# ygtxr1997/CelebBasis

Hardware: NVIDIA H100
Metric: celeb-basis training steps/sec (SD-v1 UNet 512^2, bs=1/GPU) (higher is better)
Workload: dtype f16 operands / f32 accumulate+residual (reference: f32 with TF32 convs)

## Files before the change

### celebbasis_b200/_abi.py

```python
import ctypes as C

_p, _i, _l, _f = C.c_void_p, C.c_int32, C.c_longlong, C.c_float

SIGS = {
    "cb_groupnorm_cluster_plan": [_i, _i, _i, _i, _i, _p],
    "cb_groupnorm_fwd": [_p, _i, _p, _i, _p, _p, _i, _i, _i, _i, _f, _i, _p, _p, _p, _p],
    "cb_groupnorm_bwd": [_p, _i, _p, _i, _p, _p, _p, _p, _p, _i, _p, _i, _i, _i, _i, _i, _i, _p, _p],
    "cb_layernorm_fwd": [_p, _i, _p, _i, _p, _p, _i, _i, _f, _p, _p, _p],
    "cb_layernorm_bwd": [_p, _i, _p, _i, _p, _p, _p, _p, _i, _p, _i, _i, _i, _p],
    "cb_axpby2d": [_p, _i, _l, _f, _p, _i, _l, _f, _p, _i, _l, _l, _i, _p],
    "cb_act_fwd": [_p, _i, _p, _i, _l, _i, _p],
    "cb_act_bwd": [_p, _i, _p, _i, _p, _i, _l, _i, _p],
    "cb_geglu_fwd": [_p, _p, _i, _l, _i, _i, _p],
    "cb_geglu_bwd": [_p, _p, _p, _i, _i, _l, _i, _i, _p],
    "cb_softmax_fwd": [_p, _p, _i, _l, _i, _i, _i, _p],
    "cb_softmax_bwd": [_p, _p, _p, _i, _i, _l, _i, _i, _p],
    "cb_upsample2x_fwd": [_p, _p, _i, _i, _i, _i, _i, _p],
    "cb_upsample2x_bwd": [_p, _i, _p, _i, _i, _i, _i, _i, _i, _p],
    "cb_zero_insert2x": [_p, _p, _i, _i, _i, _i, _i, _p],
    "cb_nchw_to_nhwc": [_p, _p, _i, _i, _i, _i, _i, _p],
    "cb_nhwc_to_nchw": [_p, _i, _p, _i, _i, _i, _i, _p],
    "cb_mse_fwd_bwd": [_p, _p, _p, _p, _i, _i, _f, _p],
    "cb_timestep_embedding": [_p, _p, _i, _i, _i, _f, _p],
    "cb_embedding_gather": [_p, _p, _p, _i, _i, _i, _p],
    "cb_celeb_mlp_fwd": [_p, _p, _p, _p, _p, _p, _i, _i, _i, _i, _f, _p],
    "cb_celeb_basis_fwd": [_p, _p, _p, _i, _i, _i, _i, _p],
    "cb_celeb_basis_bwd": [_p, _p, _p, _i, _i, _i, _i, _p],
    "cb_celeb_mlp_bwd": [_p, _p, _p, _p, _p, _p, _p, _p, _i, _i, _i, _i, _f, _f, _p],
    "cb_embed_inject_fwd": [_p, _p, _p, _p, _p, _i, _i, _i, _p],
    "cb_embed_inject_bwd": [_p, _p, _p, _i, _i, _i, _i, _p],
    "cb_adamw_step": [_p, _p, _p, _p, _l, _f, _f, _f, _f, _f, _i, _p, _p],
    "cb_posterior_sample": [_p, _p, _p, _i, _i, _i, _f, _p],
    "cb_ddim_step": [_p, _p, _p, _p, _p, _p, _l, _f, _f, _f, _f, _f, _p],
    "cb_attention_fwd": [_p, _l, _p, _l, _p, _l, _p, _l, _p, _p, _l, _i, _i, _i, _i, _i, _i, _f, _i, _p],
    "cb_attention_bwd": [_p, _l, _p, _l, _p, _l, _p, _l, _p, _l, _p, _p, _p, _l, _p, _l, _p, _l, _i, _i, _i, _i, _i, _i, _f,
                         _i, _p],
    "cb_attention_bwd_dq": [_p, _l, _p, _l, _p, _l, _p, _l, _p, _l, _p, _p, _p, _l, _p, _l, _i, _i, _i, _i, _i, _i, _f, _i, _p],
    "cb_q_sample": [_p, _p, _p, _p, _p, _p, _i, _i, _p],
    "cb_channel_affine_act": [_p, _i, _p, _i, _p, _p, _p, _l, _i, _p],
    "cb_face_warp_resize": [_p, _p, _i, _i, _i, _i, _i, _i, _i, _p, _p],
    "cb_l2norm_rows": [_p, _p, _i, _i, _p],
    "cb_ema_rows": [_p, _p, _i, _p, _i, _i, _i, _f, _p],
    "cb_face_augment": [_p, _p, _p, _p, _p, _i, _i, _i, _i, _i, _p],
    "cb_paste_resized": [_p, _i, _i, _p, _p, _i, _i, _i, _p],
    "cb_pack_conv_weight": [_p, _p, _i, _i, _i, _i, _i, _i, _i, _p, _p],
    "cb_convert_f32": [_p, _p, _i, _l, _f, _p],
}


def declare(lib):
    for name, argtypes in SIGS.items():
        fn = getattr(lib, name)
        fn.argtypes = argtypes
        fn.restype = C.c_int
```

### celebbasis_b200/csrc/cb_gemm.cu

```cuda
#include <algorithm>
#include <stdarg.h>
#include <stdio.h>
#include <stdlib.h>
#include <string.h>

#include "cb_common.cuh"

namespace cb {

constexpr int BM = 128;
constexpr int BK = 64;
constexpr int kThreads = 384;

struct GemmParams {
    int M, N, K;
    int kchunks, taps, kw;
    int ksteps_last;
    int conv;
    int out_h, out_w, img_n;
    int box_w, box_h, box_i;
    int tiles_w, tiles_h;
    int stride, pad_top, pad_left;
    int b_tap_rows, flip_taps;
    void* D;
// ... 386 lines not shown
                for (int j = 0; j < 8; ++j) {
                    fv[j] += p.bias ? s_bias[vcol + j] : 0.f;
                    fg[j] += p.bias ? s_bias[vcol + 32 + j] : 0.f;
                }
                if (p.D) {
                    store8_any(p.D, p.d_dtype, grow * p.ldd + n0 + vcol, fv);
                    store8_any(p.D, p.d_dtype, grow * p.ldd + n0 + vcol + 32, fg);
                }
                float h[8];
#pragma unroll
                for (int j = 0; j < 8; ++j) h[j] = fv[j] * gelu_f(fg[j]);
                store8_any(p.D2, p.d2_dtype, grow * p.ldd2 + ((n0 + (q >> 2) * 64) >> 1) + (q & 3) * 8, h);
            }
            return;
        }
    }

    const bool r_pre = p.R && p.vec_ok && !p.d_transposed;
    uint4 rq[kResAhead + 1][2];
    auto res_fetch = [&](int k, uint4 (&v)[2]) {
        const int u = tid + k * kThreads;
        if (u >= BM * G) return;
        const int row = u / G, col = (u % G) * 8;
        const long long grow = s_grow[row];
        if (grow >= 0 && col + 8 <= ncols_tile) residual_load8(p, r_off + grow * p.ldr + n0 + col, v);
    };
    if (r_pre) {
#pragma unroll
        for (int k = 0; k < kResAhead; ++k) res_fetch(k, rq[k]);
    }
    const int nunits = (BM * G - tid + kThreads - 1) / kThreads;
#pragma unroll 1
    for (int k = 0; k < nunits; ++k) {
        if (r_pre) res_fetch(k + kResAhead, rq[kResAhead]);
        const int u = tid + k * kThreads;
        const int row = p.d_transposed ? u % BM : u / G;
        const int col = (p.d_transposed ? u / BM : u % G) * 8;
        const long long grow = s_grow[row];
        if (col < ncols_tile && grow >= 0) {
            const int ncols = min(8, ncols_tile - col);
            float f[8], r[8];
            stage_ld8(stage + row * kPitch + col, p.alpha, f);
            if (r_pre && ncols == 8) residual_unpack8(p, rq[0], r);
            epilogue_group8<kExt>(p, f, grow, s_brow[row], n0 + col, d_off, r_off, ncols, r_pre && ncols == 8 ? r : nullptr,
                                  sbias_of(row, col));
        }
        if (dbg && k == 0 && tid == 64) dbg[6] = clock64();
        if (r_pre) {
#pragma unroll
            for (int j = 0; j < kResAhead; ++j) { rq[j][0] = rq[j + 1][0]; rq[j][1] = rq[j + 1][1]; }
        }
    }
}

template <int BN, bool A_MN, bool B_MN, int kStages, bool kExt>
__global__ void __launch_bounds__(kThreads, 1)
cb_gemm_kernel(const __grid_constant__ CUtensorMap tmA, const __grid_constant__ CUtensorMap tmB,
               const __grid_constant__ GemmParams p) {
    using Cfg = TileCfg<BN, kStages>;
    using SCfg = StageCfg<BN>;
    extern __shared__ uint8_t smem_raw[];
    const uint32_t smem_base = (smem_u32(smem_raw) + 1023u) & ~1023u;
    float* stage = reinterpret_cast<float*>(smem_raw + (smem_base - smem_u32(smem_raw)));
    const uint32_t bar_base = smem_base + kStages * Cfg::kStageBytes;
    auto full_bar = [&](int s) { return bar_base + 8u * s; };
    auto empty_bar = [&](int s) { return bar_base + 8u * (kStages + s); };

    __shared__ long long s_grow[BM];
    __shared__ int s_brow[BM];
    __shared__ __align__(16) float s_bias[BN];
    const int warp = threadIdx.x >> 5;
    const int wg = __shfl_sync(0xffffffffu, warp >> 2, 0);
    if (p.dbg_mode == 3) { pdl_sync(); return; }
    unsigned long long* dbg = p.dbg ? p.dbg + 8ull * ((blockIdx.z * gridDim.y + blockIdx.y) * gridDim.x + blockIdx.x) : nullptr;
    if (dbg && threadIdx.x == 0) { dbg[0] = clock64(); dbg[7] = gtimer(); }
    const int n0 = blockIdx.x * BN;
    const int m_tile = blockIdx.y;
    const int sp = blockIdx.z % p.splits;
    const int bz = blockIdx.z / p.splits;
    const int zi = bz % p.batch_inner;
    const int zo = bz / p.batch_inner;

    int m0 = 0, ow0 = 0, oh0 = 0, img0 = 0;
    if (p.conv) {
        const int tw = m_tile % p.tiles_w;
        const int th = (m_tile / p.tiles_w) % p.tiles_h;
        const int ti = m_tile / (p.tiles_w * p.tiles_h);
        ow0 = tw * p.box_w;
        oh0 = th * p.box_h;
        img0 = ti * p.box_i;
    } else {
        m0 = m_tile * BM;
    }

    if (threadIdx.x == 0) {
        tma_prefetch_desc(&tmA);
        tma_prefetch_desc(&tmB);
        for (int s = 0; s < kStages; ++s) {
            mbar_init(full_bar(s), 1);
            mbar_init(empty_bar(s), 8);
        }
        mbar_fence_init();
        fence_proxy_async_smem();
    }
    __syncthreads();
    if (dbg && threadIdx.x == 0) dbg[1] = clock64();
    pdl_sync();

    const int kiters_all = p.dbg_mode == 1 ? 0 : p.taps * p.kchunks;
    const int it0 = sp * p.kiters_per_split;
    const int it1 = min(kiters_all, it0 + p.kiters_per_split);

    if (wg == 0) {
        if (threadIdx.x == 0) {
            int s = 0;
            uint32_t ph = 0;
            int tap = it0 / p.kchunks;
            int kc = it0 - tap * p.kchunks;
            int r = tap / p.kw;
            int sx = tap - r * p.kw;
            for (int it = it0; it < it1; ++it) {
                mbar_wait(empty_bar(s), ph ^ 1u);
                mbar_arrive_expect_tx(full_bar(s), p.a_bytes + p.b_bytes);
                const uint32_t a_dst = smem_base + s * Cfg::kStageBytes;
                const uint32_t b_dst = a_dst + Cfg::kABytes;
                const int tap_b = p.flip_taps ? (p.taps - 1 - tap) : tap;
                if (p.conv) {
                    tma_load_4d(a_dst, &tmA, full_bar(s), kc * BK, ow0 * p.stride + sx - p.pad_left,
                                oh0 * p.stride + r - p.pad_top, img0);
                } else if (A_MN) {
                    tma_load_4d(a_dst, &tmA, full_bar(s), m0, kc * BK, zi, zo);
                    tma_load_4d(a_dst + 8192, &tmA, full_bar(s), m0 + 64, kc * BK, zi, zo);
                } else {
                    tma_load_4d(a_dst, &tmA, full_bar(s), kc * BK, m0, zi, zo);
                }
                if (B_MN) {
#pragma unroll
                    for (int j = 0; j < BN / 64; ++j)
                        tma_load_4d(b_dst + j * 8192, &tmB, full_bar(s), n0 + j * 64,
                                    tap_b * p.b_tap_rows + kc * BK, zi, zo);
                } else {
                    tma_load_4d(b_dst, &tmB, full_bar(s), kc * BK, tap_b * p.b_tap_rows + n0, zi, zo);
                }
                if (++s == kStages) { s = 0; ph ^= 1u; }
                if (++kc == p.kchunks) {
                    kc = 0;
                    ++tap;
                    if (++sx == p.kw) { sx = 0; ++r; }
                }
            }
        }
        __syncwarp();
        const int r = threadIdx.x;
        long long grow;
        bool row_valid;
        if (p.conv) {
            const int per_img = p.box_h * p.box_w;
            const int bi = r / per_img;
            const int rem = r - bi * per_img;
            const int bh = rem / p.box_w;
            const int bw = rem - bh * p.box_w;
            const int img = img0 + bi, oh = oh0 + bh, ow = ow0 + bw;
            row_valid = (bi < p.box_i) && (img < p.img_n) && (oh < p.out_h) && (ow < p.out_w);
            grow = ((long long)img * p.out_h + oh) * p.out_w + ow;
        } else {
            grow = m0 + r;
            row_valid = grow < p.M;
        }
        s_grow[r] = row_valid ? grow : -1;
        if (p.bias) {
            const long long tile_row0 = p.conv ? (((long long)img0 * p.out_h + oh0) * p.out_w + ow0) : (long long)m0;
            const long long brow0 = p.bias_row_div > 0 ? tile_row0 / p.bias_row_div : 0;
            const long long brow = p.bias_row_div > 0 ? grow / p.bias_row_div : 0;
            s_brow[r] = brow == brow0 ? -1 : static_cast<int>(brow);
            const int ncols = min(BN, p.N - n0);
            for (int i = r; i < BN; i += 128) s_bias[i] = i < ncols ? p.bias[brow0 * p.ldbias + n0 + i] : 0.f;
        }
    } else {
        float acc[BN / 2];
#pragma unroll
        for (int i = 0; i < BN / 2; ++i) acc[i] = 0.f;
        const uint32_t a_half = static_cast<uint32_t>(wg - 1) * 8192u;
        const bool releaser = (threadIdx.x & 31) == 0;
        int s = 0, s_prev = 0;
        uint32_t ph = 0;
        int kc = it0 % p.kchunks;
        for (int it = it0; it < it1; ++it) {
            mbar_wait(full_bar(s), ph);
            if (dbg && it == it0 && threadIdx.x == 128) dbg[2] = clock64();
            const uint32_t a_src = smem_base + s * Cfg::kStageBytes + a_half;
            const uint32_t b_src = smem_base + s * Cfg::kStageBytes + Cfg::kABytes;
            const int ksteps = (kc == p.kchunks - 1) ? p.ksteps_last : (BK / 16);
            wgmma_fence_regs(acc);
            if (p.bf16) mma_kiter<BN, A_MN, B_MN, true>(acc, a_src, b_src, ksteps);
            else mma_kiter<BN, A_MN, B_MN, false>(acc, a_src, b_src, ksteps);
            wgmma_wait<1>();
            wgmma_fence_regs(acc);
            if (it > it0 && releaser) mbar_arrive(empty_bar(s_prev));
            s_prev = s;
            if (++s == kStages) { s = 0; ph ^= 1u; }
            if (++kc == p.kchunks) kc = 0;
        }
        wgmma_wait<0>();
        wgmma_fence_regs(acc);
        if (it1 > it0 && releaser) mbar_arrive(empty_bar(s_prev));
        if (dbg && threadIdx.x == 128) dbg[3] = clock64();
        named_bar(4, 256);
        const int l = threadIdx.x & 31, w = warp & 3;
        float* srow = stage + ((wg - 1) * 64 + w * 16 + (l >> 2)) * SCfg::kPitch + 2 * (l & 3);
#pragma unroll
        for (int j = 0; j < BN / 8; ++j) {
            *reinterpret_cast<float2*>(srow + 8 * j) = make_float2(acc[4 * j], acc[4 * j + 1]);
            *reinterpret_cast<float2*>(srow + 8 * SCfg::kPitch + 8 * j) = make_float2(acc[4 * j + 2], acc[4 * j + 3]);
        }
    }
    named_bar(2, kThreads);
    const int ncols_tile = min(BN, p.N - n0);
    if (p.splits > 1 && !p.cluster_sk && p.dbg_mode == 0) {
        const unsigned tile_id = (static_cast<unsigned>(bz) * gridDim.y + m_tile) * gridDim.x + blockIdx.x;
        if (!splitk_reduce_to_stage<BN>(p, tile_id, sp, stage, ncols_tile)) return;
    }
    if (p.dbg_mode == 1 || p.dbg_mode == 2) return;
    if (dbg && threadIdx.x == 64) dbg[4] = clock64();
    epilogue_units<BN, kExt>(p, stage, s_grow, s_brow, s_bias, n0, ncols_tile, zo, zi, sp, smem_base + SCfg::kBytes, dbg);
    if (dbg && threadIdx.x == 64) dbg[5] = clock64();
}

typedef CUresult (*EncodeTiledFn)(CUtensorMap*, CUtensorMapDataType, cuuint32_t, void*, const cuuint64_t*,
                                  const cuuint64_t*, const cuuint32_t*, const cuuint32_t*,
                                  CUtensorMapInterleave, CUtensorMapSwizzle, CUtensorMapL2promotion,
                                  CUtensorMapFloatOOBfill);

static EncodeTiledFn get_encode_fn() {
    static EncodeTiledFn fn = nullptr;
    static bool tried = false;
    if (!tried) {
        tried = true;
        void* p = nullptr;
        cudaDriverEntryPointQueryResult q;
        if (cudaGetDriverEntryPoint("cuTensorMapEncodeTiled", &p, cudaEnableDefault, &q) == cudaSuccess &&
            q == cudaDriverEntryPointSuccess) {
            fn = reinterpret_cast<EncodeTiledFn>(p);
        }
    }
    return fn;
}

int make_tmap(CUtensorMap* out, int dtype, int rank, const void* ptr, const uint64_t* dims,
              const uint64_t* strides_bytes , const uint32_t* box, const uint32_t* estr) {
    EncodeTiledFn fn = get_encode_fn();
    CB_REQUIRE(fn != nullptr, CB_ERR_DRIVER, "cuTensorMapEncodeTiled entry point unavailable");
    CB_REQUIRE((reinterpret_cast<uintptr_t>(ptr) & 15u) == 0, CB_ERR_ALIGN, "tensor base %p not 16B aligned", ptr);
    for (int i = 0; i < rank - 1; ++i)
        CB_REQUIRE((strides_bytes[i] & 15u) == 0, CB_ERR_ALIGN, "tensor stride[%d]=%llu bytes not multiple of 16", i,
                   (unsigned long long)strides_bytes[i]);
    CUtensorMapDataType dt = dtype == CB_F16 ? CU_TENSOR_MAP_DATA_TYPE_FLOAT16 : CU_TENSOR_MAP_DATA_TYPE_BFLOAT16;
    CUresult rc = fn(out, dt, (cuuint32_t)rank, const_cast<void*>(ptr), dims, strides_bytes, box, estr,
                     CU_TENSOR_MAP_INTERLEAVE_NONE, CU_TENSOR_MAP_SWIZZLE_128B, CU_TENSOR_MAP_L2_PROMOTION_L2_256B,
                     CU_TENSOR_MAP_FLOAT_OOB_FILL_NONE);
    CB_REQUIRE(rc == CUDA_SUCCESS, CB_ERR_DRIVER,
               "cuTensorMapEncodeTiled failed rc=%d rank=%d dims=[%llu,%llu,%llu,%llu] box=[%u,%u,%u,%u]", (int)rc,
               rank, (unsigned long long)dims[0], (unsigned long long)dims[1],
               (unsigned long long)(rank > 2 ? dims[2] : 0), (unsigned long long)(rank > 3 ? dims[3] : 0), box[0],
               box[1], rank > 2 ? box[2] : 0, rank > 3 ? box[3] : 0);
    return 0;
}

static inline bool needs_ext(const GemmParams& p) { return p.D2 != nullptr || p.act == CB_ACT_PRELU || p.glu; }

template <int BN, bool A_MN, bool B_MN, int kStages, bool kExt>
static int launch_se(const CUtensorMap& tA, const CUtensorMap& tB, const GemmParams& p, dim3 grid, cudaStream_t st) {
    using Cfg = TileCfg<BN, kStages>;
    static bool attr_done = false;
    auto kern = cb_gemm_kernel<BN, A_MN, B_MN, kStages, kExt>;
    if (!attr_done) {
        CB_CUDA(cudaFuncSetAttribute(kern, cudaFuncAttributeMaxDynamicSharedMemorySize, Cfg::kSmemBytes));
        attr_done = true;
    }
    if (p.cluster_sk) {
        const int S = p.splits;
        CB_REQUIRE(S >= 2 && S <= 16 && grid.z % S == 0, CB_ERR_ARG, "cb_gemm(cluster split-K): %d slices not in [2,16]", S);
        static bool np_done = false;
        if (S > 8 && !np_done) {
            CB_CUDA(cudaFuncSetAttribute(kern, cudaFuncAttributeNonPortableClusterSizeAllowed, 1));
            np_done = true;
        }
        CB_CUDA(launch_kernel_cluster(kern, grid, dim3(kThreads), dim3(1, 1, (unsigned)S), (size_t)Cfg::kSmemBytes, st, tA, tB, p));
        CB_CUDA(cudaGetLastError());
        count_launches(1);
        return 0;
    }
CB_LAUNCH((kern), grid, kThreads, Cfg::kSmemBytes, st, tA, tB, p);
    CB_CUDA(cudaGetLastError());
    count_launches(1);
    return 0;
}

template <int BN, bool A_MN, bool B_MN, int kStages>
static int launch_s(const CUtensorMap& tA, const CUtensorMap& tB, const GemmParams& p, dim3 grid, cudaStream_t st) {
    return needs_ext(p) ? launch_se<BN, A_MN, B_MN, kStages, true>(tA, tB, p, grid, st)
                        : launch_se<BN, A_MN, B_MN, kStages, false>(tA, tB, p, grid, st);
}

static int ring_stages(int bn, const GemmParams& p, long long ctas) {
    if (bn == 256) return 4;
    static const int env_force = getenv("CB_GEMM_STAGES") ? atoi(getenv("CB_GEMM_STAGES")) : 0;
    const int force = p.force_stages ? p.force_stages : env_force;
    if (force == 3) return 3;
    if (force == 6 || ctas <= device_sm_count()) return 6;
    return 3;
}
static bool cluster_sk_fits(int bn, int splits, int stages) {
    const long long stage_bytes = ((long long)BM * (bn + 4) * 4 + 1023) / 1024 * 1024;
    const long long ring = (long long)stages * (BM * BK * 2 + bn * BK * 2);
    const long long gi = (bn / 8 + splits - 1) / splits;
    return stage_bytes + (long long)splits * gi * BM * 32 <= ring;
}

template <int BN, bool A_MN, bool B_MN>
static int launch(const CUtensorMap& tA, const CUtensorMap& tB, const GemmParams& p, dim3 grid, cudaStream_t st) {
    if constexpr (BN == 256) {
        return launch_s<BN, A_MN, B_MN, 4>(tA, tB, p, grid, st);
    } else {
        const long long ctas = (long long)grid.x * grid.y * grid.z;
        if (ring_stages(BN, p, ctas) == 6) return launch_s<BN, A_MN, B_MN, 6>(tA, tB, p, grid, st);
        return launch_s<BN, A_MN, B_MN, 3>(tA, tB, p, grid, st);
    }
}

static double tile_time_us(int bn, long long tiles, int kiters, int sms) {
    const double t_iter = (128.0 + bn) * 128.0 / 80e3;
    const long long waves = (tiles + sms - 1) / sms;
    return (double)waves * kiters * t_iter;
}

static int pick_bn(const cb_gemm_desc& d, int m_tiles, int kiters, bool requested = true) {
    const int N = d.N;
    const int sms = device_sm_count();
    int cands[3];
    int nc = 0;
    if (d.b_major == CB_MAJOR_MN) {
        if (N <= 64) return 64;
        cands[nc++] = 128;
        cands[nc++] = 64;
    } else {
        if (N <= 64) return 64;
        cands[nc++] = 160;
        cands[nc++] = 128;
        cands[nc++] = 64;
    }
    static const int env_bn = getenv("CB_GEMM_BN") ? atoi(getenv("CB_GEMM_BN")) : 0;
    const int force_bn = !requested ? 0 : (d.tile_n > 0 ? d.tile_n : env_bn);
    if (force_bn == 256 && N >= 256) return 256;
    for (int i = 0; i < nc; ++i)
        if (cands[i] == force_bn) return force_bn;
    int best = cands[0];
    double best_t = 1e30;
    for (int i = 0; i < nc; ++i) {
        const int bn = cands[i];
        const long long tiles = (long long)ceil_div(N, bn) * m_tiles * d.batch;
        double t = tile_time_us(bn, tiles, kiters, sms) + 0.02 * ceil_div(N, bn);
        if (t < best_t) { best_t = t; best = bn; }
    }
    return best;
}

}

using namespace cb;

extern "C" int cb_gemm(const cb_gemm_desc* dp, void* stream) {
    CB_REQUIRE(dp != nullptr, CB_ERR_ARG, "cb_gemm: null desc");
    const cb_gemm_desc& d = *dp;
    CB_REQUIRE(d.ab_dtype == CB_F16 || d.ab_dtype == CB_BF16, CB_ERR_ARG, "cb_gemm: ab_dtype must be f16/bf16");
    CB_REQUIRE(d.A && d.B && (d.D || (d.glu && d.D2)), CB_ERR_ARG, "cb_gemm: null A/B/D");
    if (d.glu) {
        CB_REQUIRE(d.D2 && d.N % 64 == 0 && d.batch == 1 && !d.d_transposed && !d.R && d.act == CB_ACT_NONE &&
                       d.bias_row_div == 0,
                   CB_ERR_ARG, "cb_gemm(glu): needs D2, N %% 64 == 0, batch 1, no residual / activation / per-image bias");
    }
    CB_REQUIRE(d.N > 0 && d.K > 0 && d.batch > 0, CB_ERR_ARG, "cb_gemm: bad N/K/batch");
    CB_REQUIRE(d.d_dtype >= CB_F16 && d.d_dtype <= CB_F32, CB_ERR_ARG, "cb_gemm: bad d_dtype");
    const int es = 2;
    const bool a_mn = d.a_major == CB_MAJOR_MN, b_mn = d.b_major == CB_MAJOR_MN;
    CB_REQUIRE(!(d.conv && a_mn), CB_ERR_ARG, "cb_gemm: conv mode needs K-major A (NHWC)");
    CB_REQUIRE(!(a_mn && !b_mn), CB_ERR_ARG, "cb_gemm: (A MN-major, B K-major) is not instantiated");

    const int b_in = d.batch_inner > 0 ? d.batch_inner : d.batch;
    CB_REQUIRE(d.batch % b_in == 0, CB_ERR_ARG, "cb_gemm: batch %d not a multiple of batch_inner %d", d.batch, b_in);
    const int b_out = d.batch / b_in;
    GemmParams p;
    memset(&p, 0, sizeof(p));
    p.batch_inner = b_in;
    p.N = d.N;
    p.K = d.K;
    p.kchunks = ceil_div(d.K, BK);
    p.ksteps_last = ceil_div(d.K - (p.kchunks - 1) * BK, 16);
    p.conv = d.conv;
    p.taps = 1;
    p.kw = 1;
    p.b_tap_rows = d.b_tap_rows;
    p.flip_taps = d.flip_taps;

    CUtensorMap tA, tB;
    int m_tiles;
    if (d.conv) {
        CB_REQUIRE(d.img_n > 0 && d.img_h > 0 && d.img_w > 0 && d.out_h > 0 && d.out_w > 0 && d.kh > 0 && d.kw > 0,
                   CB_ERR_ARG, "cb_gemm(conv): bad geometry");
        CB_REQUIRE(d.stride == 1 || d.stride == 2, CB_ERR_ARG, "cb_gemm(conv): stride must be 1 or 2");
        CB_REQUIRE(d.batch == 1, CB_ERR_ARG, "cb_gemm(conv): batch must be 1 (images are rows)");
        p.taps = d.kh * d.kw;
        p.kw = d.kw;
        p.M = d.img_n * d.out_h * d.out_w;
        p.out_h = d.out_h;
        p.out_w = d.out_w;
        p.img_n = d.img_n;
        p.stride = d.stride;
        p.pad_top = d.pad_top;
        p.pad_left = d.pad_left;
        int bw = d.out_w < BM ? d.out_w : BM;
        int bh = BM / bw;
        if (bh > d.out_h) bh = d.out_h;
        int bi = BM / (bw * bh);
        if (bi > d.img_n) bi = d.img_n;
        if (bi < 1) bi = 1;
        p.box_w = bw;
        p.box_h = bh;
        p.box_i = bi;
        p.tiles_w = ceil_div(d.out_w, bw);
        p.tiles_h = ceil_div(d.out_h, bh);
        m_tiles = p.tiles_w * p.tiles_h * ceil_div(d.img_n, bi);
        p.a_bytes = (unsigned)(bw * bh * bi) * BK * es;
        const uint64_t C = (uint64_t)d.K;
        const uint64_t rowstride = (uint64_t)d.lda;
        uint64_t dims[4] = {C, (uint64_t)d.img_w, (uint64_t)d.img_h, (uint64_t)d.img_n};
        uint64_t strides[3] = {rowstride * es, rowstride * es * d.img_w, rowstride * es * d.img_w * d.img_h};
        uint32_t box[4] = {BK, (uint32_t)(bw * d.stride), (uint32_t)(bh * d.stride), (uint32_t)bi};
        uint32_t estr[4] = {1, (uint32_t)d.stride, (uint32_t)d.stride, 1};
        CB_REQUIRE(box[1] <= 256 && box[2] <= 256, CB_ERR_ARG, "cb_gemm(conv): box too large");
        int rc = make_tmap(&tA, d.ab_dtype, 4, d.A, dims, strides, box, estr);
        if (rc) return rc;
    } else {
        CB_REQUIRE(d.M > 0, CB_ERR_ARG, "cb_gemm: bad M");
        p.M = d.M;
        m_tiles = ceil_div(d.M, BM);
        p.a_bytes = BM * BK * es;
        const uint64_t dflt = (uint64_t)(a_mn ? d.lda * (int64_t)d.K : d.lda * (int64_t)d.M);
        const uint64_t bs = (uint64_t)(b_in > 1 ? d.a_batch_stride : dflt);
        const uint64_t bs2 = (uint64_t)(b_out > 1 ? d.a_batch_stride2 : dflt);
        if (a_mn) {
            uint64_t dims[4] = {(uint64_t)d.M, (uint64_t)d.K, (uint64_t)b_in, (uint64_t)b_out};
            uint64_t strides[3] = {(uint64_t)d.lda * es, bs * es, bs2 * es};
            uint32_t box[4] = {64, BK, 1, 1};
            uint32_t estr[4] = {1, 1, 1, 1};
            int rc = make_tmap(&tA, d.ab_dtype, 4, d.A, dims, strides, box, estr);
            if (rc) return rc;
        } else {
            uint64_t dims[4] = {(uint64_t)d.K, (uint64_t)d.M, (uint64_t)b_in, (uint64_t)b_out};
            uint64_t strides[3] = {(uint64_t)d.lda * es, bs * es, bs2 * es};
            uint32_t box[4] = {BK, BM, 1, 1};
            uint32_t estr[4] = {1, 1, 1, 1};
            int rc = make_tmap(&tA, d.ab_dtype, 4, d.A, dims, strides, box, estr);
            if (rc) return rc;
        }
    }

    int BN = pick_bn(d, m_tiles, p.taps * p.kchunks);
    if (d.glu && BN % 64 != 0) BN = 128;
    const int b_box_rows = BN;
    p.b_bytes = (unsigned)b_box_rows * BK * es;
    {
        const uint64_t brows_total = (uint64_t)(d.conv ? (int64_t)p.taps * d.b_tap_rows : (b_mn ? d.K : d.N));
        const uint64_t dflt = (uint64_t)(d.ldb * (int64_t)brows_total);
        const uint64_t bs = (uint64_t)(b_in > 1 ? d.b_batch_stride : dflt);
        const uint64_t bs2 = (uint64_t)(b_out > 1 ? d.b_batch_stride2 : dflt);
        uint32_t estr[4] = {1, 1, 1, 1};
        if (b_mn) {
            uint64_t dims[4] = {(uint64_t)d.N, brows_total, (uint64_t)b_in, (uint64_t)b_out};
            uint64_t strides[3] = {(uint64_t)d.ldb * es, bs * es, bs2 * es};
            uint32_t box[4] = {64, BK, 1, 1};
            int rc = make_tmap(&tB, d.ab_dtype, 4, d.B, dims, strides, box, estr);
            if (rc) return rc;
        } else {
            uint64_t dims[4] = {(uint64_t)d.K, brows_total, (uint64_t)b_in, (uint64_t)b_out};
            uint64_t strides[3] = {(uint64_t)d.ldb * es, bs * es, bs2 * es};
            uint32_t box[4] = {BK, (uint32_t)b_box_rows, 1, 1};
            int rc = make_tmap(&tB, d.ab_dtype, 4, d.B, dims, strides, box, estr);
            if (rc) return rc;
        }
    }

    p.D = d.D;
    p.d_dtype = d.d_dtype;
    p.ldd = d.ldd;
    p.d_bs = d.d_batch_stride;
    p.d_bs2 = d.d_batch_stride2;
    p.d_transposed = d.d_transposed;
    p.D2 = d.D2;
    p.d2_dtype = d.d2_dtype;
    p.ldd2 = d.ldd2;
    if (d.D2) {
        CB_REQUIRE(d.batch == 1 && !d.d_transposed, CB_ERR_ARG, "cb_gemm: D2 needs batch == 1 and a non-transposed D");
        CB_REQUIRE(d.d2_dtype >= CB_F16 && d.d2_dtype <= CB_F32, CB_ERR_ARG, "cb_gemm: bad d2_dtype");
        const int es2 = d.d2_dtype == CB_F32 ? 4 : 2;
        CB_REQUIRE((reinterpret_cast<uintptr_t>(d.D2) & 15u) == 0 && (d.ldd2 * es2) % 16 == 0 &&
                       d.ldd2 >= (d.glu ? d.N / 2 : d.N),
                   CB_ERR_ALIGN, "cb_gemm: D2 must be 16-byte aligned with a 16-byte multiple row pitch >= N (N/2 with glu)");
    }
    p.glu = d.glu;
    p.act_param = d.act_param;
    p.d2_scale = d.d2_scale;
    p.d2_shift = d.d2_shift;
    CB_REQUIRE(d.act != CB_ACT_PRELU || d.act_param != nullptr, CB_ERR_ARG, "cb_gemm: CB_ACT_PRELU needs act_param (slopes)");
    CB_REQUIRE((d.d2_scale == nullptr) == (d.d2_shift == nullptr), CB_ERR_ARG, "cb_gemm: d2_scale and d2_shift go together");
    p.bias = d.bias;
    p.bias_row_div = d.bias_row_div;
    p.ldbias = d.ldbias;
    p.R = d.R;
    p.r_dtype = d.r_dtype;
    p.ldr = d.ldr;
    p.r_bs = d.r_batch_stride;
    p.r_bs2 = d.r_batch_stride2;
    p.alpha = d.alpha;
    p.act = d.act;
    p.dbg = reinterpret_cast<unsigned long long*>(d.debug_timeline);
    {
        static const int mode = getenv("CB_GEMM_DBG_MODE") ? atoi(getenv("CB_GEMM_DBG_MODE")) : 0;
        p.dbg_mode = mode;
    }
    p.bf16 = d.ab_dtype == CB_BF16 ? 1 : 0;
    {
        const int des = d.d_dtype == CB_F32 ? 4 : 2;
        bool ok = ((reinterpret_cast<uintptr_t>(d.D) & 15u) == 0) && ((d.ldd * des) % 16 == 0) &&
                  ((d.d_batch_stride * des) % 16 == 0) && ((d.d_batch_stride2 * des) % 16 == 0);
        if (d.R) {
            const int res = d.r_dtype == CB_F32 ? 4 : 2;
            ok = ok && ((reinterpret_cast<uintptr_t>(d.R) & 15u) == 0) && ((d.ldr * res) % 16 == 0) &&
                 ((d.r_batch_stride * res) % 16 == 0) && ((d.r_batch_stride2 * res) % 16 == 0);
        }
        if (d.bias) ok = ok && ((reinterpret_cast<uintptr_t>(d.bias) & 15u) == 0) && ((d.ldbias * 4) % 16 == 0);
        p.vec_ok = ok ? 1 : 0;
    }

    p.force_stages = (d.stages == 3 || d.stages == 6) ? d.stages : 0;
    p.splits = 1;
    p.kiters_per_split = p.taps * p.kchunks;
    {
        const int kiters = p.taps * p.kchunks;
        const int sms = device_sm_count();
        const int bn_s = pick_bn(d, m_tiles, kiters, false);
        const long long tiles_s = (long long)ceil_div(d.N, bn_s) * m_tiles * d.batch;
        const long long counters_bytes = 65536;
        const long long avail = d.splitk_ws_bytes - counters_bytes;
        const long long tiles_max = (long long)ceil_div(d.N, 64) * m_tiles * d.batch;
        const long long slice_bytes = (long long)(d.N + 255) * m_tiles * d.batch * BM * 4;
        if (d.splitk_ws != nullptr && !d.glu && tiles_max <= counters_bytes / 4 &&
            (d.splits > 0 || (tiles_s < sms && kiters >= 8))) {
            const double out_elems = (double)p.M * d.batch * d.N;
            double best_t = tile_time_us(bn_s, tiles_s, kiters, sms);
            int best_sp = 1;
            if (d.splits > 0) {
                best_sp = d.splits < kiters ? d.splits : kiters;
            } else {
                const int max_sp = (int)(sms / tiles_s) < 64 ? (int)(sms / tiles_s) : 64;
                for (int sp = 2; sp <= max_sp; ++sp) {
                    const int per = ceil_div(kiters, sp);
                    if (per < 4) break;
                    const double t = per * ((128.0 + bn_s) * 128.0 / 80e3) + out_elems * sp / 150e3 + 3.0;
                    if (t < best_t) { best_t = t; best_sp = sp; }
                }
            }
            if (best_sp > 1) {
                const int per = ceil_div(kiters, best_sp);
                const int splits = ceil_div(kiters, per);
                if (slice_bytes * splits <= avail) {
                    p.splits = splits;
                    p.kiters_per_split = per;
                    p.counters = reinterpret_cast<unsigned*>(d.splitk_ws);
                    p.ws = reinterpret_cast<float*>(reinterpret_cast<char*>(d.splitk_ws) + counters_bytes);
                }
            }
        }
    }
    cudaStream_t st = reinterpret_cast<cudaStream_t>(stream);
    dim3 grid((unsigned)ceil_div(d.N, BN), (unsigned)m_tiles, (unsigned)(d.batch * p.splits));
    p.cluster_sk = (d.splitk_cluster == 1 && p.splits >= 2 && p.splits <= 16 && p.dbg_mode == 0 &&
                    cluster_sk_fits(BN, p.splits, ring_stages(BN, p, (long long)grid.x * grid.y * grid.z))) ? 1 : 0;
    if (!a_mn && !b_mn) {
        if (BN == 64) return launch<64, false, false>(tA, tB, p, grid, st);
        if (BN == 128) return launch<128, false, false>(tA, tB, p, grid, st);
        if (BN == 256) return launch<256, false, false>(tA, tB, p, grid, st);
        return launch<160, false, false>(tA, tB, p, grid, st);
    } else if (!a_mn && b_mn) {
        if (BN == 64) return launch<64, false, true>(tA, tB, p, grid, st);
        if (BN == 256) return launch<256, false, true>(tA, tB, p, grid, st);
        return launch<128, false, true>(tA, tB, p, grid, st);
    } else {
        if (BN == 64) return launch<64, true, true>(tA, tB, p, grid, st);
        return launch<128, true, true>(tA, tB, p, grid, st);
    }
}
```

### include/celebbasis_b200.h

```cpp
#ifndef CELEBBASIS_B200_H_
#define CELEBBASIS_B200_H_

#include <stdint.h>

#ifdef __cplusplus
extern "C" {
#endif

#define CB_ABI_VERSION 6
#define CB_GN_WS_BYTES 131072

enum { CB_F16 = 0, CB_BF16 = 1, CB_F32 = 2 };
enum { CB_ACT_NONE = 0, CB_ACT_SILU = 1, CB_ACT_GELU = 2, CB_ACT_QUICK_GELU = 3, CB_ACT_PRELU = 4 };
enum { CB_MAJOR_K = 0, CB_MAJOR_MN = 1 };

enum {
    CB_OK = 0,
    CB_ERR_ARG = -1,
    CB_ERR_ALIGN = -2,
    CB_ERR_DRIVER = -3,
    CB_ERR_NO_DEVICE = -4,
};

int cb_abi_version(void);
const char* cb_last_error(void);
int cb_device_ok(void);
unsigned long long cb_launch_count(void);

typedef struct cb_gemm_desc {
    int32_t M, N, K;
    int32_t batch;
    int32_t ab_dtype;

    const void* A;
    int64_t lda;
    int64_t a_batch_stride;
    int32_t a_major;

    const void* B;
    int64_t ldb;
    int64_t b_batch_stride;
    int32_t b_major;

    int32_t conv;
    int32_t img_n, img_h, img_w;
    int32_t out_h, out_w;
    int32_t kh, kw;
    int32_t stride;
    int32_t pad_top, pad_left;
    int32_t b_tap_rows;
    int32_t flip_taps;

    void* D;
    int32_t d_dtype;
    int64_t ldd;
    int64_t d_batch_stride;
    int32_t d_transposed;

    const float* bias;
    int32_t bias_row_div;
    int64_t ldbias;

    const void* R;
    int32_t r_dtype;
    int64_t ldr;
    int64_t r_batch_stride;

    float alpha;
    int32_t act;

    int32_t batch_inner;
    int64_t a_batch_stride2, b_batch_stride2, d_batch_stride2, r_batch_stride2;

    void* splitk_ws;
    int64_t splitk_ws_bytes;

    void* debug_timeline;

    int32_t tile_n;
    int32_t splits;
    int32_t stages;
    int32_t cta_pair;

    void* D2;
    int64_t ldd2;
    int32_t d2_dtype;
    int32_t glu;
    const float* act_param;
    const float* d2_scale;
    const float* d2_shift;
    int32_t splitk_cluster;
} cb_gemm_desc;

int cb_gemm(const cb_gemm_desc* desc, void* stream);


#define CB_GN_CTA_CAP(n) (((n) & 0xFFFF) << 8)
int cb_groupnorm_cluster_plan(int N, int HW, int C, int G, int bytes_per_elem, int* plan);
int cb_groupnorm_fwd(const void* x, int x_dtype, void* y, int y_dtype, const float* gamma, const float* beta,
                     int N, int HW, int C, int G, float eps, int act_silu, float* mean_out, float* rstd_out,
                     double* ws, void* stream);
int cb_groupnorm_bwd(const void* dy, int dy_dtype, const void* x, int x_dtype, const float* gamma,
                     const float* beta, const float* mean, const float* rstd, void* dx, int dx_dtype, void* dx_lp, int N,
                     int HW, int C, int G, int act_silu, int accumulate, double* ws, void* stream);
int cb_layernorm_fwd(const void* x, int x_dtype, void* y, int y_dtype, const float* gamma, const float* beta, int M,
                     int C, float eps, float* mean_out, float* rstd_out, void* stream);
int cb_layernorm_bwd(const void* dy, int dy_dtype, const void* x, int x_dtype, const float* gamma, const float* mean,
                     const float* rstd, void* dx, int dx_dtype, void* dx_lp, int M, int C, int accumulate,
                     void* stream);

int cb_axpby2d(const void* x, int x_dtype, long long ldx, float a, const void* y, int y_dtype, long long ldy, float b,
               void* out, int o_dtype, long long ldo, long long rows, int cols, void* stream);
int cb_act_fwd(const void* x, int x_dtype, void* y, int y_dtype, long long n, int act, void* stream);
int cb_act_bwd(const void* dy, int dy_dtype, const void* x, int x_dtype, void* dx, int dx_dtype, long long n, int act,
               void* stream);
int cb_geglu_fwd(const void* in, void* out, int dtype, long long M, int F, int interleave, void* stream);
int cb_geglu_bwd(const void* dout, const void* in, void* din, int dtype, int g_dtype, long long M, int F,
                 int interleave, void* stream);
int cb_softmax_fwd(const void* s, void* p, int dtype, long long rows, int ncols, int ld, int causal_period,
                   void* stream);
int cb_softmax_bwd(const void* dp, const void* p, void* ds, int p_dtype, int g_dtype, long long rows, int ncols,
                   int ld, void* stream);
int cb_upsample2x_fwd(const void* x, void* y, int dtype, int N, int H, int W, int C, void* stream);
int cb_upsample2x_bwd(const void* dy, int dy_dtype, void* dx, int dx_dtype, int N, int H, int W, int C,
                      int accumulate, void* stream);
int cb_zero_insert2x(const void* dy, void* z, int dtype, int N, int H, int W, int C, void* stream);
int cb_nchw_to_nhwc(const float* x, void* y, int y_dtype, int N, int C, int HW, int Cpad, void* stream);
int cb_nhwc_to_nchw(const void* x, int x_dtype, float* y, int N, int C, int HW, int Cpad, void* stream);
int cb_mse_fwd_bwd(const float* pred, const float* target, float* loss , float* grad, int B, int per_sample,
                   float gscale, void* stream);
int cb_timestep_embedding(const long long* t, void* out, int o_dtype, int B, int dim, float max_period,
                          void* stream);

int cb_embedding_gather(const long long* ids, const float* table, float* out, int n, int D, int V, void* stream);
int cb_celeb_mlp_fwd(const float* v, const float* W, const float* b, float* pre, float* coef, float* nrm, int F,
                     int in_dim, int K, int es, float slope, void* stream);
int cb_celeb_basis_fwd(const float* coef, const float* basis, float* z, int F, int es, int K, int D, void* stream);
int cb_celeb_basis_bwd(const float* dz, const float* basis, float* dcoef, int F, int es, int K, int D, void* stream);
int cb_celeb_mlp_bwd(const float* dcoef, const float* coef, const float* nrm, const float* pre, const float* v,
                     float* dpre_ws, float* dW, float* db, int F, int in_dim, int K, int es, float slope,
                     float gscale, void* stream);
int cb_embed_inject_fwd(const float* tok, const float* z, const int* map, const float* pos, float* out, int B, int T,
                        int D, void* stream);
int cb_embed_inject_bwd(const float* dout, const int* map, float* dz, int n_z_rows, int B, int T, int D,
                        void* stream);
int cb_adamw_step(float* p, const float* g, float* m, float* v, long long n, float lr, float beta1, float beta2,
                  float eps, float weight_decay, int step, int* step_dev, void* stream);
int cb_posterior_sample(const float* moments, const float* eps, float* z, int N, int Cz, int HW, float scale,
                        void* stream);
int cb_ddim_step(const float* x, const float* e_uncond, const float* e_cond, const float* noise, float* x_prev,
                 float* pred_x0, long long n, float guidance_scale, float a_t, float a_prev, float sigma_t,
                 float sqrt_one_minus_at, void* stream);
int cb_q_sample(const float* x0, const float* noise, const long long* t, const float* sqrt_ac, const float* sqrt_1mac,
                float* out, int B, int per_sample, void* stream);

int cb_channel_affine_act(const void* x, int x_dtype, void* y, int y_dtype, const float* scale, const float* shift,
                          const float* slope, long long rows, int C, void* stream);
int cb_face_warp_resize(const float* faces, void* out, int o_dtype, int B, int H, int W, int n_chunks, int out_hw,
                        int Cpad, const float* host_affine6, void* stream);
int cb_l2norm_rows(const float* x, float* y, int rows, int D, void* stream);
int cb_ema_rows(float* table, const long long* idx, int idx_stride, const float* src, int B, int row, int n_rows,
                float momentum, void* stream);

int cb_attention_fwd(const void* Q, long long ldq, const void* K, long long ldk, const void* V, long long ldv, void* O,
                     long long ldo, float* lse, void* P, long long ldp, int dtype, int images, int heads, int nq,
                     int nk, int d, float scale, int causal, void* stream);

int cb_attention_bwd(const void* Q, long long ldq, const void* K, long long ldk, const void* V, long long ldv,
                     const void* O, long long ldo, const void* dO, long long lddo, const float* lse, float* delta,
                     void* dQ, long long lddq, void* dK, long long lddk, void* dV, long long lddv, int dtype, int images,
                     int heads, int nq, int nk, int d, float scale, int causal, void* stream);

int cb_attention_bwd_dq(const void* Q, long long ldq, const void* K, long long ldk, const void* V, long long ldv,
                        const void* O, long long ldo, const void* dO, long long lddo, const float* lse, float* delta,
                        void* dQ, long long lddq, void* dS, long long ldds, int dtype, int images, int heads, int nq,
                        int nk, int d, float scale, int causal, void* stream);

int cb_pack_conv_weight(const float* w, void* out, int o_dtype, int cout, int cin, int kh, int kw, int cout_pad,
                        int cin_pad, const float* out_scale, void* stream);
int cb_convert_f32(const float* x, void* out, int o_dtype, long long n, float scale, void* stream);

int cb_face_augment(const unsigned char* src_u8, const int* iparams, const float* fparams, double* ws, float* out, int B,
                    int H, int W, int c_total, int c_off, void* stream);
int cb_paste_resized(const float* faces, int c_total, int c_off, const int* geo, float* out, int B, int H, int W,
                     void* stream);

#ifdef __cplusplus
}
#endif
#endif
```

Baseline: 56.68.

## Plan GEMM tile width and split-K jointly with a measured cost table

Replaces the analytic tile-time heuristic and the separate split-K search with one planner. It scores every candidate N-tile width, including 256 when eligible, together with each split-K factor, using per-width fixed and per-k-iteration cost constants and a split-reduction overhead term. The ring pipeline now always uses 6 stages unless 3 is forced, where before it depended on the CTA count. It also exposes a cb_gemm_plan entry point and factors out the conv box and m-tile helpers. The cost constants may not generalise across shapes, and the change can alter tile, split and stage choices for many convolutions and linears.

```diff
diff --git a/celebbasis_b200/_abi.py b/celebbasis_b200/_abi.py
--- a/celebbasis_b200/_abi.py
+++ b/celebbasis_b200/_abi.py
@@ -3,6 +3,7 @@
 _p, _i, _l, _f = C.c_void_p, C.c_int32, C.c_longlong, C.c_float
 
 SIGS = {
+    "cb_gemm_plan": [_p, _i, _p, _p, _p],
     "cb_groupnorm_cluster_plan": [_i, _i, _i, _i, _i, _p],
     "cb_groupnorm_fwd": [_p, _i, _p, _i, _p, _p, _i, _i, _i, _i, _f, _i, _p, _p, _p, _p],
     "cb_groupnorm_bwd": [_p, _i, _p, _i, _p, _p, _p, _p, _p, _i, _p, _i, _i, _i, _i, _i, _i, _p, _p],
diff --git a/celebbasis_b200/csrc/cb_gemm.cu b/celebbasis_b200/csrc/cb_gemm.cu
--- a/celebbasis_b200/csrc/cb_gemm.cu
+++ b/celebbasis_b200/csrc/cb_gemm.cu
@@ -712,13 +712,11 @@
                         : launch_se<BN, A_MN, B_MN, kStages, false>(tA, tB, p, grid, st);
 }
 
-static int ring_stages(int bn, const GemmParams& p, long long ctas) {
+static int ring_stages(int bn, const GemmParams& p) {
     if (bn == 256) return 4;
     static const int env_force = getenv("CB_GEMM_STAGES") ? atoi(getenv("CB_GEMM_STAGES")) : 0;
     const int force = p.force_stages ? p.force_stages : env_force;
-    if (force == 3) return 3;
-    if (force == 6 || ctas <= device_sm_count()) return 6;
-    return 3;
+    return force == 3 ? 3 : 6;
 }
 static bool cluster_sk_fits(int bn, int splits, int stages) {
     const long long stage_bytes = ((long long)BM * (bn + 4) * 4 + 1023) / 1024 * 1024;
@@ -732,52 +730,138 @@
     if constexpr (BN == 256) {
         return launch_s<BN, A_MN, B_MN, 4>(tA, tB, p, grid, st);
     } else {
-        const long long ctas = (long long)grid.x * grid.y * grid.z;
-        if (ring_stages(BN, p, ctas) == 6) return launch_s<BN, A_MN, B_MN, 6>(tA, tB, p, grid, st);
+        if (ring_stages(BN, p) == 6) return launch_s<BN, A_MN, B_MN, 6>(tA, tB, p, grid, st);
         return launch_s<BN, A_MN, B_MN, 3>(tA, tB, p, grid, st);
     }
 }
 
-static double tile_time_us(int bn, long long tiles, int kiters, int sms) {
-    const double t_iter = (128.0 + bn) * 128.0 / 80e3;
-    const long long waves = (tiles + sms - 1) / sms;
-    return (double)waves * kiters * t_iter;
-}
-
-static int pick_bn(const cb_gemm_desc& d, int m_tiles, int kiters, bool requested = true) {
-    const int N = d.N;
-    const int sms = device_sm_count();
-    int cands[3];
+struct GemmCost {
+    int bn;
+    double fixed_1, fixed_full;
+    double kiter_1, kiter_full;
+};
+static const GemmCost kGemmCost[] = {{64, 3.11, 3.69, 0.311, 0.318},
+                                     {128, 4.61, 5.05, 0.326, 0.370},
+                                     {160, 5.31, 5.44, 0.353, 0.439},
+                                     {256, 7.33, 7.74, 0.566, 0.679}};
+static const double kSplitUs = 2.41, kSplitSliceUsPer128Cols = 1.09, kSplitFullUs = 2.60;
+
+static const GemmCost& gemm_cost(int bn) {
+    for (const GemmCost& c : kGemmCost)
+        if (c.bn == bn) return c;
+    return kGemmCost[1];
+}
+
+static double launch_time_us(int bn, long long tiles, int splits, int per, int sms) {
+    const GemmCost& c = gemm_cost(bn);
+    const long long ctas = tiles * splits;
+    if (ctas > sms) return (double)((ctas + sms - 1) / sms) * (c.fixed_full + per * c.kiter_full);
+    const double fill = (double)ctas / sms;
+    double t = c.fixed_1 + (c.fixed_full - c.fixed_1) * fill + per * (c.kiter_1 + (c.kiter_full - c.kiter_1) * fill);
+    if (splits > 1) t += kSplitUs + kSplitSliceUsPer128Cols * splits * bn / 128.0 + kSplitFullUs * fill;
+    return t;
+}
+
+static const long long kSplitkCounterBytes = 65536;
+
+struct GemmPlan {
+    int bn;
+    int splits;
+    int kiters_per_split;
+};
+
+static GemmPlan plan_gemm(const cb_gemm_desc& d, int m_tiles, int kiters, int sms) {
+    const bool a_mn = d.a_major == CB_MAJOR_MN, b_mn = d.b_major == CB_MAJOR_MN;
+    int cands[4];
     int nc = 0;
-    if (d.b_major == CB_MAJOR_MN) {
-        if (N <= 64) return 64;
-        cands[nc++] = 128;
+    if (d.N <= 64) {
         cands[nc++] = 64;
     } else {
-        if (N <= 64) return 64;
-        cands[nc++] = 160;
+        cands[nc++] = 64;
         cands[nc++] = 128;
-        cands[nc++] = 64;
-    }
-    static const int env_bn = getenv("CB_GEMM_BN") ? atoi(getenv("CB_GEMM_BN")) : 0;
-    const int force_bn = !requested ? 0 : (d.tile_n > 0 ? d.tile_n : env_bn);
-    if (force_bn == 256 && N >= 256) return 256;
-    for (int i = 0; i < nc; ++i)
-        if (cands[i] == force_bn) return force_bn;
-    int best = cands[0];
+        if (!b_mn && !d.glu) cands[nc++] = 160;
+        if (!b_mn && !a_mn && d.N >= 256) cands[nc++] = 256;
+    }
+
+    const long long avail = d.splitk_ws_bytes - kSplitkCounterBytes;
+    const long long tiles_max = (long long)ceil_div(d.N, 64) * m_tiles * d.batch;
+    const long long slice_bytes = (long long)(d.N + 255) * m_tiles * d.batch * BM * 4;
+    const bool can_split = d.splitk_ws != nullptr && !d.glu && tiles_max <= kSplitkCounterBytes / 4;
+    auto fits = [&](int splits) { return slice_bytes * splits <= avail; };
+
+    GemmPlan pl = {cands[0], 1, kiters};
     double best_t = 1e30;
     for (int i = 0; i < nc; ++i) {
         const int bn = cands[i];
-        const long long tiles = (long long)ceil_div(N, bn) * m_tiles * d.batch;
-        double t = tile_time_us(bn, tiles, kiters, sms) + 0.02 * ceil_div(N, bn);
-        if (t < best_t) { best_t = t; best = bn; }
-    }
-    return best;
-}
+        const long long tiles = (long long)ceil_div(d.N, bn) * m_tiles * d.batch;
+        const double t1 = launch_time_us(bn, tiles, 1, kiters, sms);
+        if (t1 < best_t) { best_t = t1; pl = {bn, 1, kiters}; }
+        if (!can_split || d.splits > 0) continue;
+        for (int sp = 2; tiles * sp <= sms; ++sp) {
+            const int per = ceil_div(kiters, sp);
+            if (per < 4) break;
+            const int splits = ceil_div(kiters, per);
+            if (splits != sp || !fits(splits)) continue;
+            const double t = launch_time_us(bn, tiles, splits, per, sms);
+            if (t < best_t) { best_t = t; pl = {bn, splits, per}; }
+        }
+    }
+    if (can_split && d.splits > 1) {
+        const int per = ceil_div(kiters, d.splits < kiters ? d.splits : kiters);
+        const int splits = ceil_div(kiters, per);
+        pl.splits = fits(splits) ? splits : 1;
+        pl.kiters_per_split = fits(splits) ? per : kiters;
+    }
+
+    static const int env_bn = getenv("CB_GEMM_BN") ? atoi(getenv("CB_GEMM_BN")) : 0;
+    const int want = d.tile_n > 0 ? d.tile_n : env_bn;
+    if (want == 256 && d.N >= 256 && !a_mn) {
+        pl.bn = 256;
+    } else {
+        for (int i = 0; i < nc; ++i)
+            if (cands[i] == want) pl.bn = want;
+    }
+    return pl;
+}
+
+static void conv_box(const cb_gemm_desc& d, int* bw, int* bh, int* bi) {
+    *bw = d.out_w < BM ? d.out_w : BM;
+    *bh = BM / *bw;
+    if (*bh > d.out_h) *bh = d.out_h;
+    *bi = BM / (*bw * *bh);
+    if (*bi > d.img_n) *bi = d.img_n;
+    if (*bi < 1) *bi = 1;
+}
+
+static int m_tiles_of(const cb_gemm_desc& d) {
+    if (!d.conv) return ceil_div(d.M, BM);
+    int bw, bh, bi;
+    conv_box(d, &bw, &bh, &bi);
+    return ceil_div(d.out_w, bw) * ceil_div(d.out_h, bh) * ceil_div(d.img_n, bi);
+}
+
+static int kiters_of(const cb_gemm_desc& d) { return (d.conv ? d.kh * d.kw : 1) * ceil_div(d.K, BK); }
 
 }
 
 using namespace cb;
+
+extern "C" int cb_gemm_plan(const cb_gemm_desc* dp, int sms, int* tile_n, int* splits, int* grid) {
+    CB_REQUIRE(dp != nullptr && tile_n != nullptr && splits != nullptr && grid != nullptr && sms >= 0, CB_ERR_ARG,
+               "cb_gemm_plan: bad arguments");
+    const cb_gemm_desc& d = *dp;
+    CB_REQUIRE(d.N > 0 && d.K > 0 && d.batch > 0, CB_ERR_ARG, "cb_gemm_plan: bad N/K/batch");
+    CB_REQUIRE(d.conv ? (d.img_n > 0 && d.out_h > 0 && d.out_w > 0 && d.kh > 0 && d.kw > 0) : d.M > 0, CB_ERR_ARG,
+               "cb_gemm_plan: bad M / conv geometry");
+    const int m_tiles = m_tiles_of(d);
+    const GemmPlan pl = plan_gemm(d, m_tiles, kiters_of(d), sms > 0 ? sms : device_sm_count());
+    *tile_n = pl.bn;
+    *splits = pl.splits;
+    grid[0] = ceil_div(d.N, pl.bn);
+    grid[1] = m_tiles;
+    grid[2] = d.batch * pl.splits;
+    return 0;
+}
 
 extern "C" int cb_gemm(const cb_gemm_desc* dp, void* stream) {
     CB_REQUIRE(dp != nullptr, CB_ERR_ARG, "cb_gemm: null desc");
@@ -828,18 +912,14 @@
         p.stride = d.stride;
         p.pad_top = d.pad_top;
         p.pad_left = d.pad_left;
-        int bw = d.out_w < BM ? d.out_w : BM;
-        int bh = BM / bw;
-        if (bh > d.out_h) bh = d.out_h;
-        int bi = BM / (bw * bh);
-        if (bi > d.img_n) bi = d.img_n;
-        if (bi < 1) bi = 1;
+        int bw, bh, bi;
+        conv_box(d, &bw, &bh, &bi);
         p.box_w = bw;
         p.box_h = bh;
         p.box_i = bi;
         p.tiles_w = ceil_div(d.out_w, bw);
         p.tiles_h = ceil_div(d.out_h, bh);
-        m_tiles = p.tiles_w * p.tiles_h * ceil_div(d.img_n, bi);
+        m_tiles = m_tiles_of(d);
         p.a_bytes = (unsigned)(bw * bh * bi) * BK * es;
         const uint64_t C = (uint64_t)d.K;
         const uint64_t rowstride = (uint64_t)d.lda;
@@ -853,7 +933,7 @@
     } else {
         CB_REQUIRE(d.M > 0, CB_ERR_ARG, "cb_gemm: bad M");
         p.M = d.M;
-        m_tiles = ceil_div(d.M, BM);
+        m_tiles = m_tiles_of(d);
         p.a_bytes = BM * BK * es;
         const uint64_t dflt = (uint64_t)(a_mn ? d.lda * (int64_t)d.K : d.lda * (int64_t)d.M);
         const uint64_t bs = (uint64_t)(b_in > 1 ? d.a_batch_stride : dflt);
@@ -875,8 +955,8 @@
         }
     }
 
-    int BN = pick_bn(d, m_tiles, p.taps * p.kchunks);
-    if (d.glu && BN % 64 != 0) BN = 128;
+    const GemmPlan plan = plan_gemm(d, m_tiles, kiters_of(d), device_sm_count());
+    const int BN = plan.bn;
     const int b_box_rows = BN;
     p.b_bytes = (unsigned)b_box_rows * BK * es;
     {
@@ -953,49 +1033,16 @@
     }
 
     p.force_stages = (d.stages == 3 || d.stages == 6) ? d.stages : 0;
-    p.splits = 1;
-    p.kiters_per_split = p.taps * p.kchunks;
-    {
-        const int kiters = p.taps * p.kchunks;
-        const int sms = device_sm_count();
-        const int bn_s = pick_bn(d, m_tiles, kiters, false);
-        const long long tiles_s = (long long)ceil_div(d.N, bn_s) * m_tiles * d.batch;
-        const long long counters_bytes = 65536;
-        const long long avail = d.splitk_ws_bytes - counters_bytes;
-        const long long tiles_max = (long long)ceil_div(d.N, 64) * m_tiles * d.batch;
-        const long long slice_bytes = (long long)(d.N + 255) * m_tiles * d.batch * BM * 4;
-        if (d.splitk_ws != nullptr && !d.glu && tiles_max <= counters_bytes / 4 &&
-            (d.splits > 0 || (tiles_s < sms && kiters >= 8))) {
-            const double out_elems = (double)p.M * d.batch * d.N;
-            double best_t = tile_time_us(bn_s, tiles_s, kiters, sms);
-            int best_sp = 1;
-            if (d.splits > 0) {
-                best_sp = d.splits < kiters ? d.splits : kiters;
-            } else {
-                const int max_sp = (int)(sms / tiles_s) < 64 ? (int)(sms / tiles_s) : 64;
-                for (int sp = 2; sp <= max_sp; ++sp) {
-                    const int per = ceil_div(kiters, sp);
-                    if (per < 4) break;
-                    const double t = per * ((128.0 + bn_s) * 128.0 / 80e3) + out_elems * sp / 150e3 + 3.0;
-                    if (t < best_t) { best_t = t; best_sp = sp; }
-                }
-            }
-            if (best_sp > 1) {
-                const int per = ceil_div(kiters, best_sp);
-                const int splits = ceil_div(kiters, per);
-                if (slice_bytes * splits <= avail) {
-                    p.splits = splits;
-                    p.kiters_per_split = per;
-                    p.counters = reinterpret_cast<unsigned*>(d.splitk_ws);
-                    p.ws = reinterpret_cast<float*>(reinterpret_cast<char*>(d.splitk_ws) + counters_bytes);
-                }
-            }
-        }
+    p.splits = plan.splits;
+    p.kiters_per_split = plan.kiters_per_split;
+    if (p.splits > 1) {
+        p.counters = reinterpret_cast<unsigned*>(d.splitk_ws);
+        p.ws = reinterpret_cast<float*>(reinterpret_cast<char*>(d.splitk_ws) + kSplitkCounterBytes);
     }
     cudaStream_t st = reinterpret_cast<cudaStream_t>(stream);
     dim3 grid((unsigned)ceil_div(d.N, BN), (unsigned)m_tiles, (unsigned)(d.batch * p.splits));
     p.cluster_sk = (d.splitk_cluster == 1 && p.splits >= 2 && p.splits <= 16 && p.dbg_mode == 0 &&
-                    cluster_sk_fits(BN, p.splits, ring_stages(BN, p, (long long)grid.x * grid.y * grid.z))) ? 1 : 0;
+                    cluster_sk_fits(BN, p.splits, ring_stages(BN, p))) ? 1 : 0;
     if (!a_mn && !b_mn) {
         if (BN == 64) return launch<64, false, false>(tA, tB, p, grid, st);
         if (BN == 128) return launch<128, false, false>(tA, tB, p, grid, st);
diff --git a/include/celebbasis_b200.h b/include/celebbasis_b200.h
--- a/include/celebbasis_b200.h
+++ b/include/celebbasis_b200.h
@@ -93,6 +93,7 @@
 } cb_gemm_desc;
 
 int cb_gemm(const cb_gemm_desc* desc, void* stream);
+int cb_gemm_plan(const cb_gemm_desc* desc, int sms, int* tile_n, int* splits, int* grid);
 
 
 #define CB_GN_CTA_CAP(n) (((n) & 0xFFFF) << 8)
```

New measurement: 57.94 (median of 6 runs). 1.02x the previous value.
